# itsdevbear/go-avalanche

Hardware: AMD Instinct MI355X
Metric: vote-record updates/sec (node·target·round) at 1/2/4/8 GPU; % HBM roofline (higher is better)
Workload: dtype u32; 1 GPU; C4: 1M nodes x 1000 targets, k=8, Bernoulli(0.8) initial acceptance, honest, sim mode; n_nodes=1000000, n_targets=1000, k=8, parallelism=single GPU

## Files before the change

### go-avalanche_amd/csrc/engine.cpp

```cpp
#include <algorithm>
#include <cstdarg>
#include <cstdio>
#include <cstring>
#include <memory>
#include <string>
#include <utility>
#include <vector>

#include "engine.h"

using namespace aveng;

namespace aveng {

static thread_local std::string g_last_error;

int fail(int code, const char* fmt, ...) {
  char buf[512];
  va_list ap;
  va_start(ap, fmt);
  vsnprintf(buf, sizeof(buf), fmt, ap);
  va_end(ap);
  g_last_error = buf;
  return code;
}

int set_device(av_engine* e) {
  AV_CHECK(e, AV_ERR_INVALID_ARG, "null engine");
  AV_HIP(hipSetDevice(e->cfg.device));
  return AV_OK;
}

avk::RoundParams round_params(const av_engine* e, const uint32_t* replay) {
  avk::RoundParams p{};
  p.planes = e->planes;
  p.pref_in = e->pref[e->cur];
  p.pref_out = e->pref[av_engine::nxt(e->cur)];
  p.pref_prev = e->pref[av_engine::prv(e->cur)];
  p.vstale = e->vstale;
  p.valid = e->valid;
  p.byz = e->byz;
  p.replay = replay;
  p.log = e->log;
  p.log_count = e->log_count;
  p.dlog = e->dlog;
  p.dlog_count = e->dlog_count;
  p.upd_count = e->upd_count;
  p.dlog_cap = e->dlog_cap;
  p.mlog = e->mlog;
  p.mlog_count = e->mlog_count;
  p.mlog_cap = e->mlog_cap;
  p.log_overflow = e->log_overflow;
  p.applied = e->applied;
  p.bytes = e->bytes;
  p.finalized = e->finalized;
  p.warm_skip = e->facts.c_monotone ? 1u : 0u;
  p.plane_nt = e->plane_nt ? 1u : 0u;
  p.ablate_gather = e->ablate_gather ? 1u : 0u;
  p.ablate_emit = (uint32_t)e->ablate_emit;
  p.ablate_phase = e->ablate_phase;
  p.ablate_node = e->ablate_node;
  p.mat_run = e->mat_run;
  p.tile_draw = e->tile_draw;
  p.seed = e->cfg.seed;
  p.log_cap = e->log_cap;
  p.log_shards = e->log_shards;
  p.n_nodes = (uint32_t)e->N;
  p.n0 = (uint32_t)e->n0;
  p.NL = e->NL;
  p.BL = e->BL;
  p.PS = e->PS;
  p.L = e->L;
  p.Lpad = e->Lpad;
  p.t0 = (uint32_t)e->t0;
  p.round = (uint32_t)e->round;
  p.round_rel = (uint32_t)(e->round - e->log_base);
  p.round_shift = e->round_shift;
  p.peer_mode = e->cfg.peer_mode;
  p.warm_all = e->facts.warm_all ? 1u : 0u;
  p.store_policy = e->store_policy;
  p.bl_magic = e->bl_magic;
  p.bl_sh1 = e->bl_sh1;
  p.bl_sh2 = e->bl_sh2;
  p.kpend = e->kpend;
  p.tn = (uint32_t)(e->t1 - e->t0);
  p.nopipe = e->sweep_nopipe ? 1u : 0u;
  p.tpw = e->wave_runs && e->sweep_blocks ? 1u : 0u;
  p.settled_fast = e->settled_fast ? 1u : 0u;
  p.lean = e->settled_lean && 64 % e->BL == 0 ? 1u : 0u;
  p.bl_log2 = (uint32_t)__builtin_ctz(e->BL);
  p.pub_mode = (uint32_t)e->pub_mode;
  p.readd = e->pub_mode == 2 ? e->readd : nullptr;
  p.died_out = e->pub_mode == 2 ? e->died_out : nullptr;
  p.nopoll = e->any_nopoll ? e->nopoll : nullptr;
  p.dense_min = e->dense_min;
  p.wave_dense = e->wave_dense;
  p.uni_votes = e->uni_votes;
  p.quiet_tiles = e->quiet_tiles;
  return p;
}

int materialize(av_engine* e, bool votes, bool counts) {
  if (votes && e->facts.c_preset) {
    AV_HIP(avk::launch_c_unpreset(e->planes, e->BL, e->L, (uint32_t)(e->t1 - e->t0), e->stream));
    e->facts.c_unpreset();
  }
  votes = votes && e->facts.v_stale;
  counts = counts && e->facts.k_pend;
  if (!votes && !counts) return AV_OK;
  AV_HIP(avk::launch_materialize(round_params(e, nullptr), votes, counts, e->stream));
  if (votes) e->facts.votes_written_back();
  if (counts) e->facts.counts_written_back();
  return AV_OK;
}
int materialize_votes(av_engine* e) { return materialize(e, true, true); }

int engine_scratch(av_engine* e, size_t bytes, void** out) {
  const hipError_t he = e->fetch_scratch.reserve(bytes);
  AV_CHECK(he == hipSuccess, oom_or_hip(he), "scratch (%zu B): %s", bytes, hipGetErrorString(he));
  *out = e->fetch_scratch;
  return AV_OK;
}

int ref_pick(av_engine* e) {
  if (e->ref_node != -1) return AV_OK;
  e->ref_node = -2;
  const size_t words = std::min<size_t>((e->N + 31) / 32, 1024);
  std::vector<uint32_t> w(words);
  AV_HIP(hipMemcpyAsync(w.data(), e->byz, words * 4, hipMemcpyDeviceToHost, e->stream));
  AV_HIP(hipStreamSynchronize(e->stream));
  for (size_t i = 0; i < words && e->ref_node < 0; ++i)
    if (~w[i]) {
      const int64_t n = (int64_t)i * 32 + __builtin_ctz(~w[i]);
      if (n < e->N) e->ref_node = n;
    }
  return AV_OK;
}

uint32_t default_sweep_blocks(const av_engine* e, bool force) {
  if (e->k > 8 || e->capped) return 0;
  const uint64_t tiles = e->Lpad / 64;
  if (force) {
    int bpc = 0, cus = 0;
    if (avk::round_sweep_occupancy(e->k, false, &bpc, &cus) != hipSuccess || bpc <= 0 || cus <= 0) return 0;
    return (uint32_t)(bpc * cus);
  }
  uint64_t tpw = e->tiles_per_wave;
  if (!tpw && e->BL <= 8) tpw = 16;
  if (!tpw) {
    tpw = 16;
    while (tpw > 4 && (tpw > (uint64_t)e->BL || tiles / tpw < 15000)) tpw /= 2;
  }
  const uint64_t waves = (tiles + tpw - 1) / tpw;
  return (uint32_t)std::max<uint64_t>(1, (waves + 3) / 4);
}

uint64_t log_writer_waves(const av_engine* e) {
  if (e->capped) return (uint64_t)e->NL * ((e->BL + 63) / 64);
  return avk::sweep_run_waves(e->Lpad / 64, e->sweep_blocks);
}

uint64_t log_shards_for(uint64_t w) {
  uint64_t sh = 1;
  while (sh * 2 <= avk::kLogShards && sh * 2 * 4 <= w) sh *= 2;
  return sh;
}

void set_log_layout(av_engine* e) {
  e->log_shards = (uint32_t)log_shards_for(log_writer_waves(e));
  e->log_cap = (uint32_t)std::min<size_t>(e->log_alloc / e->log_shards, 0xFFFFFFFFu);
// ... 518 lines not shown
           AV_ERR_INVALID_ARG, "replay stream not prepared for these rounds");
  if (rounds > 0) e->facts.replay_call();
  const size_t per = e->round_replay_words();
  const bool fuse = e->replay_fuse > 1 && e->kernel == 2 && e->k <= 8 && e->capped && e->pub_mode == 0 &&
                    !e->any_nopoll && e->peer_world <= 1 && !e->comm && e->NL == (uint32_t)e->N;
  for (int32_t r = 0; r < rounds;) {
    const uint32_t* rp = e->replay + per * (size_t)(e->round - e->replay_first);
    const int32_t n = fuse ? std::min<int32_t>(rounds - r, e->replay_fuse) : 1;
    AV_TRY(n > 1 ? launch_replay_fused(e, rp, n) : launch_one_round(e, rp));
    r += n;
  }
  return AV_OK;
}

int av_synchronize(av_engine* e) {
  AV_ENTER(e);
  AV_HIP(hipStreamSynchronize(e->stream));
  AV_PEER_CHECK(e);
  return AV_OK;
}

int av_round_index(av_engine* e, int64_t* out) {
  AV_CHECK(e && out, AV_ERR_INVALID_ARG, "null argument");
  *out = e->round;
  return AV_OK;
}

int av_get_round(av_engine* e, int64_t node, int64_t* out) {
  AV_CHECK(e && out, AV_ERR_INVALID_ARG, "null argument");
  AV_CHECK(local_node(e, node), AV_ERR_INVALID_ARG, "node %lld not in this shard", (long long)node);
  *out = e->proc_round.empty() ? 0 : e->proc_round[(size_t)(node - e->n0)];
  return AV_OK;
}

int av_set_round(av_engine* e, int64_t node, int64_t round) {
  AV_CHECK(e, AV_ERR_INVALID_ARG, "null argument");
  AV_CHECK(local_node(e, node), AV_ERR_INVALID_ARG, "node %lld not in this shard", (long long)node);
  if (e->proc_round.empty()) e->proc_round.assign(e->NL, 0);
  e->proc_round[(size_t)(node - e->n0)] = round;
  return AV_OK;
}

int av_materialize(av_engine* e) {
  AV_ENTER(e);
  AV_PEER_CHECK(e);
  hipEvent_t ev0 = nullptr, ev1 = nullptr;
  if (e->facts.v_stale || e->facts.k_pend || e->facts.c_preset) AV_TRY(timing_begin(e, &ev0, &ev1));
  AV_TRY(materialize_votes(e));
  return ev0 ? timing_end(e, ev0, ev1) : AV_OK;
}

}

namespace {

enum OptKind { kBool, kReject, kClamp };
struct PlainOption {
  const char* name;
  OptKind kind;
  int64_t lo, hi;
  bool av_engine::*b;
  uint32_t av_engine::*u;
  int av_engine::*i;
};
constexpr PlainOption opt(const char* n, bool av_engine::*m) { return {n, kBool, 0, 1, m, nullptr, nullptr}; }
constexpr PlainOption opt(const char* n, uint32_t av_engine::*m, OptKind kd = kBool, int64_t lo = 0, int64_t hi = 1) {
  return {n, kd, lo, hi, nullptr, m, nullptr};
}
constexpr PlainOption opt(const char* n, int av_engine::*m, OptKind kd, int64_t lo, int64_t hi) {
  return {n, kd, lo, hi, nullptr, nullptr, m};
}

constexpr PlainOption kPlainOptions[] = {
    opt("plane_nt", &av_engine::plane_nt),
    opt("uniform_rows", &av_engine::uni_rows),
    opt("ref_rows", &av_engine::ref_rows),
    opt("virtual_votes", &av_engine::virtual_votes),
    opt("vv_min_bl", &av_engine::vv_min_bl, kReject, 1, (1ll << 31) - 1),
    opt("kernel", &av_engine::kernel, kReject, 1, 2),
    opt("store_policy", &av_engine::store_policy, kReject, 0, 3),
    opt("settled_fast", &av_engine::settled_fast),
    opt("settled_lean", &av_engine::settled_lean),
    opt("wave_runs", &av_engine::wave_runs),
    opt("sweep_nopipe", &av_engine::sweep_nopipe),
    opt("uni_merge", &av_engine::uni_merge, kReject, 1, 16),
    opt("uni_votes", &av_engine::uni_votes),
    opt("quiet_tiles", &av_engine::quiet_tiles),
    opt("calm_tiles", &av_engine::calm_tiles),
    opt("net_quiet", &av_engine::net_quiet),
    opt("net_quiet_group", &av_engine::nq_group, kReject, 1, 16),
    opt("net_quiet_front", &av_engine::nq_front),
    opt("wave_dense", &av_engine::wave_dense, kReject, 0, 64),
    opt("tile_draw", &av_engine::tile_draw, kReject, 0, 1),
    opt("materialize_run", &av_engine::mat_run, kReject, 1, 64),
    opt("c_preset", &av_engine::c_preset),
    opt("replay_fuse", &av_engine::replay_fuse, kReject, 0, 4096),
    opt("replay_fast", &av_engine::replay_fast),
    opt("dropin_fast", &av_engine::dropin_fast),
    opt("admit_map", &av_engine::admit_map, kReject, 0, 2),
    opt("push_defer", &av_engine::push_defer),
    opt("push_store", &av_engine::push_store, kReject, 0, 2),
    opt("census_blocks", &av_engine::census_blocks, kReject, 0, 65536),
    opt("catalog_blocks", &av_engine::catalog_blocks, kReject, 0, 65535),
    opt("catalog_lds", &av_engine::catalog_lds),
    opt("copy_blocks", &av_engine::copy_blocks, kReject, 0, 4096),
    opt("enc_buckets", &av_engine::enc_buckets, kReject, 1, 1ll << 30),
    opt("count_changed", &av_engine::count_changed),
    opt("round_marker", &av_engine::round_marker),
    opt("warm_pref", &av_engine::warm_pref),
    opt("unsynced_shard", &av_engine::unsynced_shard),
    opt("ablate_gather", &av_engine::ablate_gather),
    opt("ablate_phase", &av_engine::ablate_phase, kClamp, 0, 31),
    opt("ablate_emit", &av_engine::ablate_emit, kClamp, 0, 3),
    opt("ablate_node", &av_engine::ablate_node, kClamp, 0, 7),
};

int opt_range(const char* name, int64_t value, int64_t lo, int64_t hi) {
  AV_CHECK(value >= lo && value <= hi, AV_ERR_INVALID_ARG, "%s must be in [%lld, %lld]", name, (long long)lo,
           (long long)hi);
  return AV_OK;
}

int set_plain(av_engine* e, const PlainOption& o, int64_t value) {
  if (o.kind == kReject) AV_TRY(opt_range(o.name, value, o.lo, o.hi));
  value = o.kind == kBool ? value != 0 : std::max(o.lo, std::min(o.hi, value));
  if (o.b)
    e->*o.b = value != 0;
  else if (o.u)
    e->*o.u = (uint32_t)value;
  else
    e->*o.i = (int)value;
  return AV_OK;
}

int opt_sweep_blocks(av_engine* e, int64_t value) {
  AV_TRY(opt_range("sweep_blocks", value, -2, (1ll << 31) - 1));
  AV_ENTER(e);
  e->sweep_blocks = value < 0 ? default_sweep_blocks(e, value == -2) : (uint32_t)value;
  e->sweep_blocks_explicit = value >= 0;
  return relayout_log_if_empty(e);
}

int opt_tiles_per_wave(av_engine* e, int64_t value) {
  AV_TRY(opt_range("tiles_per_wave", value, 0, 4096));
  AV_ENTER(e);
  e->tiles_per_wave = (uint32_t)value;
  if (!e->sweep_blocks_explicit) e->sweep_blocks = default_sweep_blocks(e);
  return relayout_log_if_empty(e);
}

int opt_solo_barrier(av_engine* e, int64_t value) {
  AV_CHECK(e->peer_world <= 1 && !e->comm, AV_ERR_UNSUPPORTED, "solo_barrier: engine has an exchange");
  if (value && !e->arrive) {
    AV_ENTER(e);
    AV_TRY(alloc_arrival(e));
    e->peer_arrive.p[0] = e->arrive;
  }
  e->solo_barrier = value != 0;
  e->solo_used = e->solo_used || e->solo_barrier;
  return AV_OK;
}

template <bool av_engine::*M>
int opt_count_planes(av_engine* e, int64_t value) {
  AV_ENTER(e);
  AV_TRY(materialize(e, false, true));
// ... 127 lines not shown
```

### go-avalanche_amd/csrc/engine.h

```cpp
#pragma once

#include <hip/hip_runtime.h>
#include <rccl/rccl.h>

#include <algorithm>
#include <cstdint>
#include <cstdlib>
#include <thread>
#include <utility>
#include <vector>

#pragma GCC visibility push(default)
#include "../../include/avhip.h"
#pragma GCC visibility pop
#include "engine_mem.h"
#include "kernels.h"
#include "round_plan.h"

namespace aveng {
int fail(int code, const char* fmt, ...) __attribute__((format(printf, 2, 3)));
inline int oom_or_hip(hipError_t he) { return he == hipErrorOutOfMemory ? AV_ERR_OOM : AV_ERR_HIP; }
}

#define AV_HIP(call)                                                                                           \
// ... 15 lines not shown
  } while (0)

#define AV_ENTER(e) AV_TRY(aveng::set_device(e))

#define AV_PEER_CHECK(e) AV_TRY(aveng::peer_failed(e))

#define AV_PEER_SYNC_CHECK(e)                                      \
  do {                                                             \
    if ((e)->peer_world > 1) AV_HIP(hipStreamSynchronize((e)->stream)); \
    AV_TRY(aveng::peer_failed(e));                                 \
  } while (0)

struct PeerGroup {
  std::vector<av_engine*> members;
  avmem::Stream stream;
  int alive = 0;
};

struct av_engine {
  av_config cfg{};
  int64_t N = 0, M = 0, n0 = 0, n1 = 0, t0 = 0, t1 = 0;
  uint32_t NL = 0, BL = 0, L = 0, Lpad = 0;
  int k = 0;
  bool capped = false;
  avmem::Stream own_stream;
  hipStream_t stream = nullptr;
  avmem::DevBuf<uint32_t> planes;
  avmem::DevBuf<uint32_t> pref[3];
  uint32_t PS = 0;
  avk::RecordFacts facts;
  bool ref_rows = false;
  int64_t ref_node = -1;
  size_t rflag_off = 0;
  bool uni_rows = true;
  uint32_t uni_merge = 1;
  bool k_hi_virtual = true;
  size_t uni_off = 0;
  bool c_preset = true;

  int cur = 0;
  static int nxt(int c) { return c == 2 ? 0 : c + 1; }
  static int prv(int c) { return c == 0 ? 2 : c - 1; }
  avmem::DevBuf<uint32_t> vstale;
  avmem::DevBuf<uint32_t> kpend;
  bool count_lazy = true;
  bool virtual_votes = true;
  uint32_t vv_min_bl = 16;
  avmem::DevBuf<uint32_t> valid;
  avmem::DevBuf<uint32_t> byz;
  avmem::DevBuf<uint64_t> log;
  avmem::DevBuf<uint32_t> log_count;
  avmem::DevBuf<uint64_t> dlog;
  uint32_t* dlog_count = nullptr;
  avmem::DevBuf<uint64_t> mlog;
  uint32_t* mlog_count = nullptr;
  uint32_t mlog_cap = 0;
  avmem::DevBuf<uint32_t> upd_count;
  uint32_t dlog_cap = 0;
  avmem::DevBuf<uint32_t> log_overflow;
  avmem::DevBuf<uint32_t> node_flags;
  uint32_t log_cap = 0;
  uint32_t log_shards = 1;
  size_t log_alloc = 0, mlog_alloc = 0, dlog_alloc = 0;
  avmem::DevBuf<unsigned long long> applied;
  avmem::DevBuf<unsigned long long> bytes;
  avmem::DevBuf<unsigned long long> finalized;
  avmem::DevBuf<unsigned long long> scratch_count;
  int64_t round = 0, log_base = 0;
  uint32_t round_shift = 52;
  int64_t max_log_rounds() const { return (int64_t)1 << (64 - round_shift); }
  bool plane_nt = true;
  bool ablate_gather = false;
  uint32_t ablate_node = 0;
  int ablate_emit = 0;
  uint32_t ablate_phase = 0;
  bool unsynced_shard = false;
  bool warm_pref = false;
  avmem::DevBuf<uint32_t> touch_sink;
  int kernel = 2;
  uint32_t sweep_blocks = 0;
  bool sweep_blocks_explicit = false;
  bool sweep_nopipe = true;
  bool wave_runs = true;
  bool settled_fast = true;
  bool settled_lean = true;
  uint32_t tiles_per_wave = 0;
  uint32_t bl_magic = 1, bl_sh1 = 0, bl_sh2 = 0;
  uint32_t store_policy = 0;
  std::vector<uint32_t> valid_host;
  avmem::DevBuf<uint32_t> replay;
  int64_t replay_first = 0, replay_ready = 0;
  int replay_fuse = 16;
  bool replay_fast = true;
  bool timing = false;
  bool round_marker = false;
  avmem::Event marker;
  std::vector<std::pair<avmem::Event, avmem::Event>> events;
  double timed_ms = 0.0;
  int64_t timed_launches = 0;
  ncclComm_t comm = nullptr;
  int peer_world = 0, peer_rank = 0;
  uint32_t* peer_pref[3][avk::kMaxPeers + 1] = {};
  avmem::DevBuf<uint32_t> arrive;
  avmem::PinnedBuf<volatile uint32_t> barrier_err_host;
  uint32_t* barrier_err = nullptr;
  bool failed = false;
  bool pref_uncached = false;
  bool peer_fine = true;
  size_t pref_alloc_words = 0;
  uint32_t barrier_seq = 0;
  uint32_t barrier_timeout_ms = 30000;
  std::vector<void*> peer_opened;
  avk::PeerPtrs peer_arrive{};
  avmem::DevBuf<uint32_t*> push_tbl;
  uint64_t barrier_ticks = 0;
  bool solo_barrier = false;
  bool solo_used = false;
  PeerGroup* group = nullptr;
  bool peer_mask = true;
  bool push_defer = true;
  uint32_t push_store = 1;
  uint32_t tile_draw = 0;
  uint32_t mat_run = 1;
  uint32_t census_blocks = 0;
  bool masked = false;
  uint32_t segs = 1;
  avmem::DevBuf<uint8_t> need_mine;
  avmem::DevBuf<uint8_t> needmask;
  avmem::DevBuf<uint8_t> stale;
  uint32_t* needin = nullptr;
  avmem::DevBuf<uint32_t> needin_own;
  avk::PeerPtrs peer_needin{};
  int64_t need_ready = -1;
  int64_t need_pushed = -1;
  avmem::Stream need_stream;
  avmem::Event need_free, need_drawn;
  int64_t need_drawn_w = -1;
  avmem::DevBuf<unsigned long long> changed;
  bool count_changed = false;
  int64_t rflag_clear_round = 0;

  uint32_t dense_min = 0;
  uint32_t wave_dense = 0;
  uint32_t uni_votes = 1;
  uint32_t quiet_tiles = 1;
  uint32_t calm_tiles = 1;
  uint32_t net_quiet = 1;
  uint32_t nq_group = 16;
  uint32_t nq_front = 1;
  avmem::DevBuf<uint32_t> nq;
  int32_t pub_mode = 0;
  avmem::DevBuf<uint32_t> readd;
  avmem::DevBuf<uint32_t> died_out;
  std::vector<uint32_t> nopoll_host;
  avmem::DevBuf<uint32_t> nopoll;
  bool any_nopoll = false;
  uint32_t loss_threshold = 0;
  bool loss_neutral = false;
  std::vector<uint32_t> responding_host;
  avmem::DevBuf<uint32_t> responding;
  bool any_down = false;
  avmem::DevBuf<unsigned long long> lost;
  bool lossy() const { return loss_threshold != 0 || any_down; }
  std::vector<int64_t> proc_round;
  avmem::DevBuf<void> fetch_scratch;
  avmem::DevBuf<unsigned long long> digest;
// ... 100 lines not shown
```

### go-avalanche_amd/csrc/kernels.h

```cpp
#pragma once

#include <hip/hip_runtime.h>
#include <stdint.h>

#include <type_traits>

#include "batch_layout.h"
#include "catalog.h"

namespace avk {

constexpr int kPlanes = 25;
constexpr int kPV = 0, kPC = 8, kPA = 16, kPK = 17;
constexpr uint32_t kLogShards = 1024;
constexpr uint32_t kCtrStride = 32;
constexpr uint32_t kMaxPoll = 4096;
constexpr int kMaxK = 16;
constexpr int kMaxPeers = 15;

__host__ __device__ constexpr size_t replay_groups(int k) { return (size_t)((k + 1) / 2); }
__host__ __device__ inline size_t replay_words(uint32_t Lpad, int k) { return replay_groups(k) * 4u * Lpad; }
__host__ __device__ inline size_t replay_idx(uint32_t g, int k, int j, int c) {
  return (((size_t)(g >> 6) * replay_groups(k) + (size_t)(j >> 1)) * 64u + (g & 63u)) * 4u + (size_t)((j & 1) * 2 + c);
}

__host__ __device__ constexpr uint32_t pref_stride(uint32_t BL) {
  return BL > 32u ? (BL + 31u) / 32u * 32u : (BL <= 1u ? 1u : 1u << (32 - __builtin_clz(BL - 1u)));
}

constexpr uint32_t kPendAllLive = 0x80000000u;
constexpr uint32_t kHiVirt = 0x40000000u;
__host__ __device__ inline uint32_t real_mask(uint32_t tn, uint32_t b) {
  const uint32_t rem = tn > b * 32u ? tn - b * 32u : 0u;
  return rem >= 32u ? ~0u : ((1u << rem) - 1u);
}
constexpr uint32_t kVStale = 1u, kVUniform = 2u, kVMask = 3u, kCAll = 4u;
constexpr uint32_t kVCalm = 8u;

inline void bl_divider(uint32_t d, uint32_t& magic, uint32_t& sh1, uint32_t& sh2) {
  uint32_t l = 0;
  while ((1ull << l) < d) ++l;
  magic = (uint32_t)((((1ull << l) - d) << 32) / d + 1);
  sh1 = l < 1 ? l : 1;
  sh2 = l > 1 ? l - 1 : 0;
}

__host__ __device__ constexpr uint32_t dense_words(uint32_t k) { return (k + 5u) / 2u; }
__host__ __device__ constexpr uint32_t dense_min(uint32_t k) { return dense_words(k); }

constexpr uint32_t kMedS4Died = 1u << 8;
__host__ __device__ constexpr uint32_t med_rec_words() { return 4u; }

__host__ __device__ inline uint64_t pack_update(uint32_t round_rel, uint32_t node, uint32_t slot,
                                                uint32_t target, uint32_t status, uint32_t round_shift) {
  return ((uint64_t)round_rel << round_shift) | ((uint64_t)node << 28) | ((uint64_t)slot << 24) |
         ((uint64_t)target << 2) | (uint64_t)status;
}

constexpr uint32_t kDropUnknown = 1u << 29, kDropYes = 1u << 30, kDropCons = 1u << 31, kDropTl = (1u << 22) - 1u;
__host__ __device__ inline uint32_t dropin_word(int64_t tl, bool local, uint32_t err) {
  return (local ? (uint32_t)tl & kDropTl : kDropUnknown) | (err == 0u ? kDropYes : 0u) |
         ((int32_t)err >= 0 ? kDropCons : 0u);
}

struct RoundParams {
  uint32_t* planes;
  const uint32_t* pref_in;
  uint32_t* pref_out;
  const uint32_t* valid;
  const uint32_t* byz;
  const uint32_t* replay;
  uint64_t* log;
  uint32_t* log_count;
  uint64_t* dlog;
  uint32_t* dlog_count;
  uint32_t* upd_count;
  uint64_t* mlog;
  uint32_t* mlog_count;
  uint32_t* log_overflow;
  uint32_t* node_flags;
  uint32_t exact_rel;
  uint32_t exact_keep;
  uint32_t fuse_rounds;
  uint32_t ring_next;
  uint32_t replay_fast;
  uint64_t replay_stride;
  uint32_t* pref_ring[3];
  unsigned long long* applied;
  unsigned long long* bytes;
  unsigned long long* finalized;
  uint64_t seed;
  uint32_t log_cap;
  uint32_t dlog_cap;
  uint32_t mlog_cap;
  uint32_t log_shards;
  uint32_t n_nodes;
  uint32_t n0;
  uint32_t NL;
  uint32_t BL;
  uint32_t PS;
  uint32_t L;
  uint32_t Lpad;
  uint32_t t0;
  uint32_t round;
  uint32_t round_rel;
  uint32_t round_shift;
  int32_t peer_mode;
  uint32_t warm_skip;
  uint32_t plane_nt;
  uint32_t ablate_gather;
  uint32_t ablate_emit;
  uint32_t ablate_phase;
  uint32_t ablate_node;
  uint32_t warm_all;
  uint32_t store_policy;
  uint32_t bl_magic, bl_sh1, bl_sh2;
  uint32_t vv;
  uint32_t vv_uniform;
// ... 252 lines not shown
```

### go-avalanche_amd/csrc/sweep_kernel.h

```cpp
#pragma once
#include <hip/hip_runtime.h>

#include <algorithm>

#include "kernels.h"
#include "round_common.h"
#include "round_plan.h"
#include "round_slots.h"
#include "sweep_publish.h"
#include "sweep_tile.h"
#include "sweep_settled.h"

namespace avk {
namespace {

enum : int { kModeWarm = 0, kModeCheck = 1, kModeReplay = 2, kModeAblate = 3, kModeWarmPipe = 4, kModeFresh = 5 };

#ifndef AVK_WARM_WPE
#define AVK_WARM_WPE 5
#endif
#ifndef AVK_FRESH_WPE
#define AVK_FRESH_WPE 6
#endif
template <int K, int MODE, int POL, bool REF = false, bool CC = true>
// ... 56 lines not shown
    wd.badc = wd.badp = 0ull;
    wd.sdc = wd.sdp = nullptr;
    wd.fofs = 0u;
    uint32_t uni_done = 0u;
    bool uni_ran = false;
    __shared__ __attribute__((aligned(16))) uint32_t s_draw[4][512];
    uint32_t* const sd = s_draw[threadIdx.x >> 6];
    if constexpr (MODE == kModeWarm && K == 8) {
      if (p.tpw) {
        tile = wave0 * p.tpw;
        tile_end = min(tile + p.tpw, tiles);
        stride = 1u;
        if (p.uni_merge > 1u && p.lean && p.settled_fast && p.klazy && p.vv && p.tpw * p.uni_merge <= kUniRun &&
            uniform) {
          if (wave0 % p.uni_merge) tile = tile_end = tiles;
          else tile_end = min(tile + p.tpw * p.uni_merge, tiles);
        }
        nq_tag = tile < tiles;
        if (tile < tiles) {
          const uint32_t nlA = uni(div_bl(p, tile * 64u));
          const uint32_t nlB = uni(div_bl(p, min(tile_end * 64u, p.L) - 1u));
          const uint32_t nn = nlB - nlA + 1u;
          UniPre upre;
          const bool uni_ok = p.uni_in && p.lean && p.settled_fast && p.klazy && p.vv && nn <= 256u &&
                              tile_end - tile <= kUniRun;
          const uint32_t ti = tile + lane;
          const uint32_t st = p.vv && ti < tile_end ? p.vstale[ti] : 0u;
          const uint32_t kw = (p.klazy || p.kconsume) && ti < tile_end ? p.kpend[ti] : 0u;
          if constexpr (!CC) {
            if (uni_ok) uni_early(p, lane, nlA, upre);
          }
          wd.meta = (st << 8) | (kw & (kPendAllLive | kHiVirt | 0xFFu));
          wd.t0 = tile;
          wd.nlA = nlA;
          wd.nn = nn;
          const uint32_t all_tiles = run_mask(tile_end - tile);
          if (uni_ok && uniform) {
            const bool qt = !CC && prev_uni && p.quiet_tiles;
            if constexpr (CC) uni_early(p, lane, nlA, upre);
            const uint32_t quiet = uni_prefetch<POL>(p, lane, tile, tile_end, nn, wd.meta, qt, upre);
            uni_done = settled_run_uni<POL, CC>(p, lane, tile, tile_end, wd.meta, nlA, nn, upre, quiet, acc);
            uni_ran = true;
            if (quiet == all_tiles && uni_done == all_tiles) nq_tag = false;
          }
          const bool any_stale = __ballot((st & kVMask) == kVStale && lane < 32u && !((uni_done >> lane) & 1u)) != 0ull;
          if (uni_done != all_tiles) {
            wd.pair = any_stale;
            wd.flagok = 0ull;
            if (any_stale && nn * 2u > 32u) {
              const PairDraw dp = single_draw(p, p.round - 1u, nlA, nn, lane);
              const PairDraw dc = single_draw(p, p.round, nlA, nn, lane);
              wd.ok = !dp.fallback && !dc.fallback;
              if (wd.ok) {
                park_draw(dp, sd, lane, p.PS * 4u);
                park_draw(dc, sd + 256, lane, p.PS * 4u);
              }
              wd.sdp = sd;
              wd.sdc = sd + 256;
              wd.badp = dp.bad;
              wd.badc = dc.bad;
            } else {
              const PairDraw d = any_stale ? pair_draw(p, p.round, nlA, nn, lane) : single_draw(p, p.round, nlA, nn, lane);
              wd.ok = !d.fallback;
              if (wd.ok) park_draw(d, sd, lane, p.PS * 4u);
              wd.sdp = sd;
              wd.sdc = any_stale ? sd + 128 : sd;
              wd.badp = d.bad & 0xFFFFFFFFull;
              wd.badc = any_stale ? d.bad >> 32 : d.bad;
              wd.fofs = any_stale ? 32u : 0u;
              if constexpr (REF) {
                if (wd.ok && p.rflag_in && p.klazy) {
                  const uint8_t tag = ref_tag(p.round);
                  uint32_t ok = 1u;
#pragma unroll
                  for (int i = 0; i < 4; ++i) ok &= p.rflag_in[d.prod[i]] == tag ? 1u : 0u;
                  wd.flagok = __ballot(ok != 0u);
                }
              }
            }
          }
        }
      }
    }
    uint32_t lean_done = uni_done;
    bool lean_ran = uni_ran;
    if constexpr (MODE == kModeWarm && K == 8) {
      if (!uni_ran && wd.ok && wd.badc == 0ull && p.lean && p.settled_fast && p.klazy && p.vv && tile < tile_end) {
        lean_done = settled_run<POL, REF, CC>(p, lane, tile_end, wd, acc);
        lean_ran = true;
      }
    }
    const uint32_t qfirst = tile, qstep = stride;
    uint32_t qn = 0;
    if constexpr (MODE == kModeWarm && K == 8) {
      if (lean_ran && stride == 1u && tile < tile_end &&
          lean_done == run_mask(tile_end - tile)) {
        qn = tile_end - tile;
        tile = tile_end;
      }
    }
    const bool tdraw = MODE == kModeWarm && K == 8 && p.tile_draw && p.tpw && !wd.ok && tile < tile_end;
    for (; tile < tile_end; tile += stride) {
      constexpr bool AB = MODE == kModeAblate;
      if constexpr (CC) acc.qslot = qn++;
      if constexpr (MODE == kModeWarm) {
        if constexpr (K == 8) {
          if (lean_done && ((lean_done >> (tile - wd.t0)) & 1u)) continue;
          if (tdraw) {
            const uint32_t tnlA = uni(div_bl(p, tile * 64u));
            const uint32_t tnn = uni(div_bl(p, min(tile * 64u + 64u, p.L) - 1u)) - tnlA + 1u;
            const bool tst = ((meta_of(wd, tile) >> 8) & kVMask) == kVStale;
            const PairDraw d = tst ? pair_draw(p, p.round, tnlA, tnn, lane) : single_draw(p, p.round, tnlA, tnn, lane);
            wd.ok = !d.fallback;
            if (wd.ok) {
              park_draw(d, sd, lane, p.PS * 4u);
              wd.nlA = tnlA;
              wd.nn = tnn;
              wd.pair = tst;
              wd.sdp = sd;
              wd.sdc = tst ? sd + 128 : sd;
              wd.badp = d.bad & 0xFFFFFFFFull;
              wd.badc = tst ? d.bad >> 32 : d.bad;
              wd.fofs = tst ? 32u : 0u;
              wd.flagok = 0ull;
            }
          }
          if (wd.ok && p.settled_fast && p.klazy && p.vv && !lean_ran) {
            const uint32_t m = meta_of(wd, tile);
            const bool cok = p.calm && ((m >> 8) & kVCalm) &&
                             __ballot(lane < wd.nn && is_byz(p.byz, p.n0 + wd.nlA + lane)) == 0ull;
            if (settled_cand(m, cok ? 1u : 0u) &&
                settled_tile<POL, REF, CC>(p, tile, lane, m & (kPendAllLive | kHiVirt | 0xFFu), wd, acc, m >> 8))
              continue;
          }
        }
        TileIn<K, false, true> in;
        load_tile<K, false, true, POL, false, true, false, CC>(p, tile, lane, in, &wd, uflags);
        process_tile<K, false, true, POL, true, REF, CC, true>(p, tile, lane, in, 0u, acc, uflags);
      } else if constexpr (MODE == kModeFresh) {
        TileIn<K, false, false> in;
        load_tile<K, false, false, POL, false, true, true>(p, tile, lane, in);
        process_tile<K, false, false, POL, true>(p, tile, lane, in, 0u, acc);
      } else if constexpr (MODE == kModeReplay) {
        TileIn<K, true, false> in;
        load_tile<K, true, false, POL, false>(p, tile, lane, in);
        process_tile<K, true, false, POL>(p, tile, lane, in, 0u, acc);
      } else {
        bool warm = false;
        if (p.warm_skip) {
          const uint32_t g = tile * 64u + lane;
          const uint32_t c7 = g < p.L ? p.planes[(size_t)tile * (kPlanes * 64u) + 1024u + 7u * 64u + lane] : ~0u;
          warm = __all(c7 == ~0u);
        }
        if (warm) {
          TileIn<K, false, true> in;
          load_tile<K, false, true, POL, AB>(p, tile, lane, in);
          process_tile<K, false, true, POL>(p, tile, lane, in, 4u, acc);
        } else {
          TileIn<K, false, false> in;
          load_tile<K, false, false, POL, AB>(p, tile, lane, in);
          process_tile<K, false, false, POL>(p, tile, lane, in, 0u, acc);
        }
      }
    }
    if constexpr (CC) {
      if (p.push_q && qn) acc.pushed += (uint32_t)wave_sum(flush_pushes(p, lane, qfirst, qstep, qn, acc.qpub, acc.qpm));
    }
  }
  const unsigned long long s = wave_sum(acc.applied);
  const unsigned long long f = __ballot(acc.died != 0u) ? wave_sum(acc.died) : 0ull;
  const unsigned long long by = (unsigned long long)wave_sum(acc.lane_bytes) + acc.emitted_bytes;
  const unsigned long long rr = wave_sum(acc.reread);
  if (lane == 0) {
    const uint32_t shard = acc.shard;
    if (s) atomicAdd(&p.applied[shard], s);
    if (f) atomicAdd(&p.finalized[shard], f);
    if (by) atomicAdd(&p.bytes[shard], by);
    if (rr) atomicAdd(&p.bytes[kLogShards + shard], rr);
    if (acc.updates) atomicAdd(&p.upd_count[shard], acc.updates);
  }
  if (p.count_changed && lane == 0 && acc.changed) {
    atomicAdd(&p.changed[acc.shard], (unsigned long long)acc.changed);
    atomicAdd(&p.changed[kLogShards + acc.shard], (unsigned long long)acc.changed_segs);
  }
  if (p.count_changed && lane == 0 && acc.pushed) atomicAdd(&p.changed[2 * kLogShards + acc.shard], (unsigned long long)acc.pushed);
  if (p.nq_out && nq_tag && lane == 0) *p.nq_out = p.round + 1u;
  if (p.uni_out && __ballot(acc.umis != 0u) != 0ull && lane == 0) {
    const uint32_t tag = p.round + 1u;
    p.uni_out[p.uni_rank] = tag;
    if (!p.uni_post)
      for (uint32_t r = 0; r < p.push_n; ++r)
        __hip_atomic_store(peer_ptr(p.push_dst, r) + p.uni_off + p.uni_rank, tag, __ATOMIC_RELAXED, __HIP_MEMORY_SCOPE_SYSTEM);
  }
}

constexpr uint32_t kPushQBytes = 4u * kPushQ * 64u * 5u;

template <int K, int MODE, bool CC>
hipError_t launch_mode_cc(const RoundParams& p, uint32_t grid, hipStream_t s) {
  const uint32_t shm = CC && p.push_q ? kPushQBytes : 0u;
  const uint32_t pol = (K == 8 && p.store_policy >= 2) ? p.store_policy : (p.plane_nt ? 1u : 0u);
  if constexpr (K == 8 && MODE == kModeWarm) {
    if (p.rflag_out) {
      if (pol == 1)
        hipLaunchKernelGGL((k_round_sweep<K, MODE, 1, true, CC>), dim3(grid), dim3(256), shm, s, p);
      else
        hipLaunchKernelGGL((k_round_sweep<K, MODE, 0, true, CC>), dim3(grid), dim3(256), shm, s, p);
      return hipGetLastError();
    }
  }
  switch (pol) {
    case 0: hipLaunchKernelGGL((k_round_sweep<K, MODE, 0, false, CC>), dim3(grid), dim3(256), shm, s, p); break;
    case 1: hipLaunchKernelGGL((k_round_sweep<K, MODE, 1, false, CC>), dim3(grid), dim3(256), shm, s, p); break;
    default:
      if constexpr (K == 8) {
        if (pol == 2)
          hipLaunchKernelGGL((k_round_sweep<K, MODE, 2, false, CC>), dim3(grid), dim3(256), shm, s, p);
        else
          hipLaunchKernelGGL((k_round_sweep<K, MODE, 3, false, CC>), dim3(grid), dim3(256), shm, s, p);
      }
  }
  return hipGetLastError();
}

template <int K, int MODE>
hipError_t launch_mode(const RoundParams& p, uint32_t grid, hipStream_t s) {
  if constexpr (K == 8 && MODE == kModeWarm) {
    if (!p.count_changed) return launch_mode_cc<K, MODE, false>(p, grid, s);
  }
  return launch_mode_cc<K, MODE, true>(p, grid, s);
}

template <int K>
hipError_t launch_sweep_k(const RoundParams& p_in, SweepMode mode, uint32_t blocks, hipStream_t s, bool* ref_written) {
  if (ref_written) *ref_written = false;
  const uint32_t tiles = p_in.Lpad / 64u;
  const SweepGrid g = sweep_grid(tiles, blocks);
  RoundParams p = p_in;
  p.tpw = 0u;
  p.push_q = p.push_defer && p.push_n && p.push_n <= 8u && g.run <= kPushQ ? 1u : 0u;
  if (mode == SweepMode::Warm && p_in.tpw && K == 8 && g.run && g.run <= 16u) {
    p.tpw = g.run;
    if (ref_written) *ref_written = p.rflag_out != nullptr;
    return launch_mode<K, kModeWarm>(p, g.grid, s);
  }
  p.rflag_out = nullptr;
  p.rflag_in = nullptr;
  switch (mode) {
    case SweepMode::Replay: return launch_mode<K, kModeReplay>(p, g.grid, s);
    case SweepMode::Ablate: return launch_mode<K, kModeAblate>(p, g.grid, s);
    case SweepMode::Fresh: return launch_mode<K, kModeFresh>(p, g.grid, s);
    case SweepMode::Warm:
      if (blocks && g.grid < (tiles + 3u) / 4u && !p.nopipe) {
        p.push_q = 0u;
        return launch_mode<K, kModeWarmPipe>(p, g.grid, s);
      }
      return launch_mode<K, kModeWarm>(p, g.grid, s);
    case SweepMode::Check: break;
  }
  return launch_mode<K, kModeCheck>(p, g.grid, s);
}

template <int K>
hipError_t occupancy_k(bool replay, int* bpc) {
  return replay ? hipOccupancyMaxActiveBlocksPerMultiprocessor(bpc, k_round_sweep<K, kModeReplay, 1>, 256, 0)
                : hipOccupancyMaxActiveBlocksPerMultiprocessor(bpc, k_round_sweep<K, kModeWarmPipe, 1>, 256, 0);
}

}
}
```

### go-avalanche_amd/csrc/sweep_tile.h

```cpp
#pragma once
#include <hip/hip_runtime.h>

#include "kernels.h"
#include "round_common.h"
#include "round_slots.h"
#include "sweep_publish.h"

#ifndef AVK_ABLATE_PHASE
#define AVK_ABLATE_PHASE 0
#endif
#ifndef AVK_PUB_PRELOAD
#define AVK_PUB_PRELOAD 0
#endif

namespace avk {
namespace {

constexpr bool kAblatePhase = AVK_ABLATE_PHASE != 0;

template <int K, bool REPLAY, bool WARM>
struct TileIn {
  u32x4 v0, v1, k0, k1;
  uint32_t A, vmask, byzw;
  uint32_t stale;
// ... 80 lines not shown
      else
        in.k1 = ld4<POL>(grp + 192);
    } else {
      in.k0 = u32x4{0u, 0u, 0u, 0u};
      in.k1 = u32x4{0u, 0u, 0u, 0u};
    }
    if constexpr (!WARM) {
#pragma unroll
      for (int i = 0; i < 8; ++i) in.C[i] = ld1<POL>(tp + 1024u + (uint32_t)i * 64u + lane);
    }
  }
  in.A = kAblatePhase && VV && (p.ablate_phase & 2u) ? (lane * 0x9E3779B9u) : ld1<POL>(tp + 1536u + lane);
  if (in.stale == kVUniform) {
    in.v0 = u32x4{in.A, in.A, in.A, in.A};
    in.v1 = u32x4{in.A, in.A, in.A, in.A};
  }
  in.vmask = x.active ? p.valid[x.b] : 0u;
  in.byzw = p.byz[x.node >> 5];
  in.uref = p.uni_out ? p.pref_in[p.ref_node * p.PS + x.b] : 0u;
  in.old = 0u;
  if constexpr (REPLAY) {
    replay_load<K>(p.replay, x.gc, in.w, in.cw);
  } else {
    const uint32_t nlA = uni(x.nl), nn = (uint32_t)__builtin_amdgcn_readlane((int)x.nl, 63) - nlA + 1u;
    uint32_t peers[K];
    const uint32_t rb = p.PS * 4u, bo = x.b * 4u;
    uint32_t rows[K];
    bool drawn = false, have_rows = false;
    if constexpr (VV) {
      if (wd && wd->ok) {
        const uint32_t base = (x.nl - wd->nlA) * 2u;
        const bool nog = kAblatePhase && (p.ablate_phase & 1u);
        if (in.stale == kVStale && (uflags & kUniPrev)) {
          const uint32_t rp = at_byte(p.pref_prev, p.ref_node * rb + bo);
          in.v0 = u32x4{rp, rp, rp, rp};
          in.v1 = u32x4{rp, rp, rp, 0u};
        } else if (in.stale == kVStale) {
          uint32_t pp[K];
          pick_parked(p, wd->sdp, wd->badp, base, x.node, p.round - 1u, rb, pp);
#pragma unroll
          for (int i = 0; i < 4; ++i) in.v0[i] = nog ? pp[7 - i] * 0x9E3779B9u : at_byte(p.pref_prev, pp[7 - i] + bo);
#pragma unroll
          for (int i = 0; i < 3; ++i) in.v1[i] = nog ? pp[3 - i] * 0x9E3779B9u : at_byte(p.pref_prev, pp[3 - i] + bo);
          in.v1[3] = 0u;
        }
        pick_parked(p, wd->sdc, wd->badc, base, x.node, p.round, rb, rows);
        drawn = have_rows = true;
        if (nog) {
#pragma unroll
          for (int j = 0; j < K; ++j) in.w[j] = (rows[j] + bo) * 0x9E3779B9u;
          return;
        }
      } else if (in.stale == kVStale) {
        const PairDraw pd = pair_draw(p, p.round, nlA, nn, lane);
        {
          uint32_t pp[K];
          pick_peers(p, pd, 0u, p.round, x.node, x.nl, nlA, nn, lane, pp);
#pragma unroll
          for (int i = 0; i < 4; ++i) in.v0[i] = p.pref_prev[pp[7 - i] * p.PS + x.b];
#pragma unroll
          for (int i = 0; i < 3; ++i) in.v1[i] = p.pref_prev[pp[3 - i] * p.PS + x.b];
          in.v1[3] = 0u;
        }
        pick_peers(p, pd, 1u, p.round, x.node, x.nl, nlA, nn, lane, peers);
        drawn = true;
      }
    }
    if (uflags & kUniVotes) {
      const uint32_t rw = at_byte(p.pref_prev, p.ref_node * rb + bo);
#pragma unroll
      for (int j = 0; j < K; ++j) in.w[j] = rw;
      return;
    }
    if (!drawn) draw_peers<K>(p, p.round, x.node, x.nl, nlA, nn, lane, peers);
    if (!have_rows) {
#pragma unroll
      for (int j = 0; j < K; ++j) rows[j] = (ABLATE ? x.node : peers[j]) * rb;
    }
#pragma unroll
    for (int j = 0; j < K; ++j) in.w[j] = at_byte(p.pref_in, rows[j] + bo);
  }
}

template <int K, bool REPLAY, bool WARM, int POL, bool VVM = false, bool REF = false, bool CC = true, bool CALM = false>
__device__ __forceinline__ void process_tile(const RoundParams& p, uint32_t tile, uint32_t lane,
                                             const TileIn<K, REPLAY, WARM>& in, uint32_t extra_bytes, SweepAcc& acc,
                                             uint32_t uflags = 0u) {
  const LaneIdx x = lane_idx(p, tile, lane);
  const bool active = x.active;
  const uint32_t b = x.b, node = x.node;
  const bool nbyz = ((in.byzw >> (node & 31u)) & 1u) != 0u;
  uint32_t* const tp = p.planes + (size_t)tile * (kPlanes * 64u);
  u32x4* const grp = reinterpret_cast<u32x4*>(tp) + lane;
  const __amdgpu_buffer_rsrc_t tr = __builtin_amdgcn_make_buffer_rsrc(tp, 0, kPlanes * 64 * 4, kRsrcWord3);
  const u32x4 v0 = in.v0, v1 = in.v1;
  u32x4 k0 = in.k0, k1 = in.k1;
  uint32_t A = in.A;
  uint32_t C[8];
#pragma unroll
  for (int i = 0; i < 8; ++i) C[i] = WARM ? ~0u : in.C[WARM ? 0 : i];
  const uint32_t vmask = in.vmask;

  constexpr bool SYM = WARM && !REPLAY;
  uint32_t ys[7 + K], ns[7 + K], cwv[K];
#pragma unroll
  for (int j = 0; j < K; ++j) {
    const uint32_t cw = REPLAY ? in.cw[REPLAY ? j : 0] : ~0u;
    const uint32_t yw = in.w[j] & cw;
    ys[7 + j] = yw;
    ns[7 + j] = SYM ? 0u : ~yw & cw;
    cwv[j] = cw;
  }
#pragma unroll
  for (int i = 0; i < 7; ++i) {
    const uint32_t vi = (6 - i) < 4 ? v0[6 - i] : v1[2 - i];
    ys[i] = WARM ? vi : (vi & C[6 - i]);
    ns[i] = SYM ? 0u : WARM ? ~vi : (~vi & C[6 - i]);
  }

  constexpr bool KL = VVM && WARM && !REPLAY && K == 8;
  const bool klazy = KL && p.klazy;
  const bool kcons = KL && p.kconsume;
  const bool kunread = klazy && (in.kw & kPendAllLive);
  const uint32_t live0 = kunread ? in.vmask : ~k1[3];
  const uint32_t P0 = live0 & vmask;
  const uint32_t keep = active ? (live0 & ~vmask) : 0u;

  bool virt = false;
  if constexpr (VVM && !REPLAY && K == 8) {
    virt = p.vv && __ballot(keep != 0u) == 0ull;
    if (virt && p.vv_uniform) {
      bool st = false;
      if constexpr (SYM) {
        if (klazy) {
          uint32_t agree = P0;
#pragma unroll
          for (int i = 0; i < 7 + K; ++i) agree &= ~(ys[i] ^ in.A);
          st = __ballot(agree != P0) == 0ull;
        }
      }
      virt = st;
    }
  }
  if (active && !virt) {
    u32x4 o0, o1;
#pragma unroll
    for (int i = 0; i < 8; ++i) {
      const uint32_t vi = i < 4 ? v0[i] : v1[i - 4];
      const uint32_t vs = i < K ? ys[6 + K - i] : (i - K < 4 ? v0[i - K] : v1[i - K - 4]);
      const uint32_t vn = (vs & P0) | (vi & keep);
      if (i < 4)
        o0[i] = vn;
      else
        o1[i - 4] = vn;
    }
    st4<POL>(tr, grp, lane * 16u, o0);
    st4<POL>(tr, grp + 64, 1024u + lane * 16u, o1);
  }
  const bool cvirt = virt && !WARM && !REPLAY && p.fresh;
  if (!WARM && active && !cvirt) {
    const uint32_t dead0 = ~(P0 | keep);
#pragma unroll
    for (int i = 0; i < 8; ++i) {
      const uint32_t cs = i < K ? cwv[K - 1 - i] : C[i - K];
      st1<POL>(tr, tp + 1024u + (uint32_t)i * 64u + lane, (1024u + (uint32_t)i * 64u + lane) * 4u,
               (cs & P0) | (C[i] & keep) | dead0);
// ... 184 lines not shown
```

Measured before the change: 35700 billion vote-record updates/s (1 update = 1 regsiterVote on a live record; k=8 per node·target·round).

## Extend per-wave tile runs to fresh sweep mode with shared peer draw

Fresh-mode sweeps at K=8 now walk a contiguous run of tiles per wave, as the warm path already does. The peer draw is done once per run and parked for all tiles in it. Per-lane valid masks and the uniform reference word are hoisted out of the per-tile loop when BL is a power of two. This cuts repeated peer-sampling work and scalar loads in fresh rounds, at the cost of a specialised load path and a possible loss of grid-stride load balance.

```diff
diff --git a/go-avalanche_amd/csrc/engine.cpp b/go-avalanche_amd/csrc/engine.cpp
--- a/go-avalanche_amd/csrc/engine.cpp
+++ b/go-avalanche_amd/csrc/engine.cpp
@@ -85,7 +85,7 @@
   p.kpend = e->kpend;
   p.tn = (uint32_t)(e->t1 - e->t0);
   p.nopipe = e->sweep_nopipe ? 1u : 0u;
-  p.tpw = e->wave_runs && e->sweep_blocks ? 1u : 0u;
+  p.tpw = e->wave_runs && e->sweep_blocks ? avk::kTpwRuns | (e->fresh_runs ? avk::kTpwFresh : 0u) : 0u;
   p.settled_fast = e->settled_fast ? 1u : 0u;
   p.lean = e->settled_lean && 64 % e->BL == 0 ? 1u : 0u;
   p.bl_log2 = (uint32_t)__builtin_ctz(e->BL);
@@ -770,6 +770,7 @@
     opt("settled_fast", &av_engine::settled_fast),
     opt("settled_lean", &av_engine::settled_lean),
     opt("wave_runs", &av_engine::wave_runs),
+    opt("fresh_runs", &av_engine::fresh_runs),
     opt("sweep_nopipe", &av_engine::sweep_nopipe),
     opt("uni_merge", &av_engine::uni_merge, kReject, 1, 16),
     opt("uni_votes", &av_engine::uni_votes),
diff --git a/go-avalanche_amd/csrc/engine.h b/go-avalanche_amd/csrc/engine.h
--- a/go-avalanche_amd/csrc/engine.h
+++ b/go-avalanche_amd/csrc/engine.h
@@ -121,6 +121,7 @@
   bool sweep_blocks_explicit = false;
   bool sweep_nopipe = true;
   bool wave_runs = true;
+  bool fresh_runs = true;
   bool settled_fast = true;
   bool settled_lean = true;
   uint32_t tiles_per_wave = 0;
diff --git a/go-avalanche_amd/csrc/kernels.h b/go-avalanche_amd/csrc/kernels.h
--- a/go-avalanche_amd/csrc/kernels.h
+++ b/go-avalanche_amd/csrc/kernels.h
@@ -34,6 +34,7 @@
   const uint32_t rem = tn > b * 32u ? tn - b * 32u : 0u;
   return rem >= 32u ? ~0u : ((1u << rem) - 1u);
 }
+constexpr uint32_t kTpwRuns = 1u, kTpwFresh = 2u;
 constexpr uint32_t kVStale = 1u, kVUniform = 2u, kVMask = 3u, kCAll = 4u;
 constexpr uint32_t kVCalm = 8u;
 
diff --git a/go-avalanche_amd/csrc/sweep_kernel.h b/go-avalanche_amd/csrc/sweep_kernel.h
--- a/go-avalanche_amd/csrc/sweep_kernel.h
+++ b/go-avalanche_amd/csrc/sweep_kernel.h
@@ -162,6 +162,34 @@
         }
       }
     }
+    FreshRun fr{0u, 0u, false};
+    if constexpr (MODE == kModeFresh && K == 8) {
+      if (p.tpw) {
+        tile = wave0 * p.tpw;
+        tile_end = min(tile + p.tpw, tiles);
+        stride = 1u;
+        nq_tag = tile < tiles;
+        if (tile < tiles) {
+          const uint32_t nlA = uni(div_bl(p, tile * 64u));
+          const uint32_t nlB = uni(div_bl(p, min(tile_end * 64u, p.L) - 1u));
+          const uint32_t nn = nlB - nlA + 1u;
+          const PairDraw d = single_draw(p, p.round, nlA, nn, lane);
+          wd.ok = !d.fallback;
+          if (wd.ok) park_draw(d, sd, lane, p.PS * 4u);
+          wd.sdc = sd;
+          wd.badc = d.bad;
+          wd.t0 = tile;
+          wd.nlA = nlA;
+          wd.nn = nn;
+          if (p.BL <= 64u && (p.BL & (p.BL - 1u)) == 0u) {
+            const uint32_t b = lane & (p.BL - 1u);
+            fr.valid = p.valid[b];
+            fr.uref = p.uni_out ? p.pref_in[p.ref_node * p.PS + b] : 0u;
+            fr.hoist = true;
+          }
+        }
+      }
+    }
     uint32_t lean_done = uni_done;
     bool lean_ran = uni_ran;
     if constexpr (MODE == kModeWarm && K == 8) {
@@ -219,7 +247,10 @@
         process_tile<K, false, true, POL, true, REF, CC, true>(p, tile, lane, in, 0u, acc, uflags);
       } else if constexpr (MODE == kModeFresh) {
         TileIn<K, false, false> in;
-        load_tile<K, false, false, POL, false, true, true>(p, tile, lane, in);
+        if constexpr (K == 8)
+          load_tile_fresh<POL>(p, tile, lane, in, wd, fr);
+        else
+          load_tile<K, false, false, POL, false, true, true>(p, tile, lane, in);
         process_tile<K, false, false, POL, true>(p, tile, lane, in, 0u, acc);
       } else if constexpr (MODE == kModeReplay) {
         TileIn<K, true, false> in;
@@ -319,13 +350,15 @@
   RoundParams p = p_in;
   p.tpw = 0u;
   p.push_q = p.push_defer && p.push_n && p.push_n <= 8u && g.run <= kPushQ ? 1u : 0u;
-  if (mode == SweepMode::Warm && p_in.tpw && K == 8 && g.run && g.run <= 16u) {
+  if (mode == SweepMode::Warm && (p_in.tpw & kTpwRuns) && K == 8 && g.run && g.run <= 16u) {
     p.tpw = g.run;
     if (ref_written) *ref_written = p.rflag_out != nullptr;
     return launch_mode<K, kModeWarm>(p, g.grid, s);
   }
   p.rflag_out = nullptr;
   p.rflag_in = nullptr;
+  if (mode == SweepMode::Fresh && (p_in.tpw & kTpwRuns) && (p_in.tpw & kTpwFresh) && K == 8 && g.run && g.run <= 16u)
+    p.tpw = g.run;
   switch (mode) {
     case SweepMode::Replay: return launch_mode<K, kModeReplay>(p, g.grid, s);
     case SweepMode::Ablate: return launch_mode<K, kModeAblate>(p, g.grid, s);
diff --git a/go-avalanche_amd/csrc/sweep_tile.h b/go-avalanche_amd/csrc/sweep_tile.h
--- a/go-avalanche_amd/csrc/sweep_tile.h
+++ b/go-avalanche_amd/csrc/sweep_tile.h
@@ -186,6 +186,47 @@
   }
 }
 
+struct FreshRun {
+  uint32_t valid, uref;
+  bool hoist;
+};
+
+template <int POL>
+__device__ __forceinline__ void load_tile_fresh(const RoundParams& p, uint32_t tile, uint32_t lane,
+                                                TileIn<8, false, false>& in, const WaveDraw& wd,
+                                                const FreshRun& fr) {
+  const LaneIdx x = lane_idx(p, tile, lane);
+  const uint32_t* const tp = p.planes + (size_t)tile * (kPlanes * 64u);
+  in.stale = in.cflag = in.kw = 0u;
+  in.v0 = in.v1 = in.k0 = u32x4{0u, 0u, 0u, 0u};
+  in.k1 = u32x4{0u, 0u, 0u, ~real_mask(p.tn, x.b)};
+#pragma unroll
+  for (int i = 0; i < 8; ++i) in.C[i] = 0u;
+  in.A = ld1<POL>(tp + 1536u + lane);
+  if (fr.hoist) {
+    in.vmask = x.active ? fr.valid : 0u;
+    in.uref = fr.uref;
+  } else {
+    in.vmask = x.active ? p.valid[x.b] : 0u;
+    in.uref = p.uni_out ? p.pref_in[p.ref_node * p.PS + x.b] : 0u;
+  }
+  in.byzw = p.byz[x.node >> 5];
+  in.old = 0u;
+  const uint32_t rb = p.PS * 4u, bo = x.b * 4u;
+  uint32_t rows[8];
+  if (wd.ok) {
+    pick_parked(p, wd.sdc, wd.badc, (x.nl - wd.nlA) * 2u, x.node, p.round, rb, rows);
+  } else {
+    const uint32_t nlA = uni(x.nl), nn = (uint32_t)__builtin_amdgcn_readlane((int)x.nl, 63) - nlA + 1u;
+    uint32_t peers[8];
+    draw_peers<8>(p, p.round, x.node, x.nl, nlA, nn, lane, peers);
+#pragma unroll
+    for (int j = 0; j < 8; ++j) rows[j] = peers[j] * rb;
+  }
+#pragma unroll
+  for (int j = 0; j < 8; ++j) in.w[j] = at_byte(p.pref_in, rows[j] + bo);
+}
+
 template <int K, bool REPLAY, bool WARM, int POL, bool VVM = false, bool REF = false, bool CC = true, bool CALM = false>
 __device__ __forceinline__ void process_tile(const RoundParams& p, uint32_t tile, uint32_t lane,
                                              const TileIn<K, REPLAY, WARM>& in, uint32_t extra_bytes, SweepAcc& acc,
```

Measured after the change: 36200 billion vote-record updates/s (1 update = 1 regsiterVote on a live record; k=8 per node·target·round) (median of 4 runs). No clear change (+1.4%).
